# LCSL/nys-koop-lqr

Measured on AMD Instinct MI355X. Metric: Nyström-Koopman fits/sec (K_nm build + A,B,C solve), N=1e5 m=2000 d=384, higher is better.
Workload: dtype f64

## Files before the change

nys_koop_lqr_amd/csrc/nk_api.hip:

```cpp
#include "nk_common.h"
#include "nk_api_internal.h"

#include <cmath>
#include <cstdarg>
#include <cstdio>
#include <cstring>
#include <cstdlib>
#include <algorithm>
#include <mutex>
#include <set>

namespace nk {

static thread_local std::string g_err;

void set_error(const char* fmt, ...) {
  char buf[1024];
  va_list ap;
  va_start(ap, fmt);
  vsnprintf(buf, sizeof(buf), fmt, ap);
  va_end(ap);
  g_err = buf;
}

// ... 334 lines not shown
  NK_TRY(launch_copy2d(ctx, a.ptr, a.ld, mdl->A, mp, m, m));
  if (p > 0) {
    NK_TRY(stage_in(ctx, B, p, m, p, &b));
    NK_TRY(launch_copy2d(ctx, b.ptr, b.ld, mdl->B, mp, m, p));
  }
  NK_TRY(stage_in(ctx, C, m, d, m, &c));
  NK_TRY(launch_copy2d(ctx, c.ptr, c.ld, mdl->C, m, d, m));
  if (W) {
    NK_TRY(stage_in(ctx, W, mp, d, mp, &w));
    NK_TRY(launch_copy2d(ctx, w.ptr, w.ld, mdl->W, mp, d, mp));
  } else {
    NK_TRY(launch_gemm(ctx, false, false, d, mp, m, 1.0, mdl->C, m, mdl->A, mp, 0.0, mdl->W, mp));
  }
  mdl->has_ops = true;
  return NK_OK;
}

static hipError_t copy_ops_block(double* dst, int64_t ldd, const double* src, int64_t lds, int64_t rows, int64_t cols,
                                 hipStream_t st) {
  const hipMemcpyKind kind = is_device_ptr(dst) ? hipMemcpyDeviceToDevice : hipMemcpyDeviceToHost;
  if (ldd == cols && lds == cols) return hipMemcpyAsync(dst, src, (size_t)rows * cols * 8, kind, st);
  return hipMemcpy2DAsync(dst, (size_t)ldd * 8, src, (size_t)lds * 8, (size_t)cols * 8, (size_t)rows, kind, st);
}

extern "C" {

int nk_version(void) { return NK_ABI_VERSION; }

const char* nk_last_error(void) { return g_err.c_str(); }

int nk_device_count(void) {
  int n = 0;
  if (hipGetDeviceCount(&n) != hipSuccess) {
    (void)hipGetLastError();
    return 0;
  }
  return n;
}

int nk_create(int device, nk_ctx** out) {
  NK_REQUIRE(out != nullptr, "nk_create: null output pointer");
  *out = nullptr;
  int n = nk_device_count();
  if (n <= 0) {
    set_error("no HIP device visible: libnyskoop has no CPU fallback");
    return NK_ERR_NO_DEVICE;
  }
  NK_REQUIRE(device >= 0 && device < n, "nk_create: device %d out of range (0..%d)", device, n - 1);
  NK_HIP(hipSetDevice(device));
  hipDeviceProp_t prop;
  NK_HIP(hipGetDeviceProperties(&prop, device));
  if (strncmp(prop.gcnArchName, "gfx950", 6) != 0) {
    set_error("device %d is %s; libnyskoop is built for gfx950 (MI355X) only", device, prop.gcnArchName);
    return NK_ERR_NO_DEVICE;
  }
  nk_ctx* ctx = new nk_ctx();
  ctx->device = device;
  ctx->num_cu = prop.multiProcessorCount;
  int prio_lo = 0, prio_hi = 0;
  NK_HIP(hipDeviceGetStreamPriorityRange(&prio_lo, &prio_hi));
  const int prio_mid = (prio_lo - prio_hi >= 2) ? (prio_lo + prio_hi) / 2 : prio_hi;
  NK_HIP(hipStreamCreateWithPriority(&ctx->stream_main, hipStreamNonBlocking, prio_mid));
  NK_HIP(hipStreamCreateWithPriority(&ctx->stream_side, hipStreamNonBlocking, prio_lo));
  NK_HIP(hipStreamCreateWithPriority(&ctx->stream_prep, hipStreamNonBlocking, prio_hi));
  NK_HIP(hipStreamCreateWithFlags(&ctx->stream_copy, hipStreamNonBlocking));
  NK_HIP(hipStreamCreateWithPriority(&ctx->stream_la[0], hipStreamNonBlocking, prio_hi));
  NK_HIP(hipStreamCreateWithPriority(&ctx->stream_la[1], hipStreamNonBlocking, prio_mid));
  for (int q = 0; q < 2; ++q)
    for (int i = 0; i < 4; ++i) NK_HIP(hipEventCreateWithFlags(&ctx->ev_la[q][i], hipEventDisableTiming));
  ctx->stream = ctx->stream_main;
  ctx->cur_arena = &ctx->arena;
  NK_HIP(hipEventCreateWithFlags(&ctx->ev_fork, hipEventDisableTiming));
  NK_HIP(hipEventCreateWithFlags(&ctx->ev_join, hipEventDisableTiming));
  NK_HIP(hipEventCreateWithFlags(&ctx->ev_chain, hipEventDisableTiming));
  NK_HIP(hipMalloc(reinterpret_cast<void**>(&ctx->d_info), 256));
  ctx->d_piv = reinterpret_cast<unsigned long long*>(ctx->d_info + 16);
  NK_HIP(hipMalloc(reinterpret_cast<void**>(&ctx->d_scalars), HS_COUNT * sizeof(double)));
  NK_HIP(hipHostMalloc(reinterpret_cast<void**>(&ctx->h_scalars), HS_COUNT * sizeof(double), hipHostMallocMapped | hipHostMallocCoherent));
  NK_HIP(hipHostMalloc(reinterpret_cast<void**>(&ctx->h_info), 256, hipHostMallocMapped | hipHostMallocCoherent));
  ctx->h_piv = reinterpret_cast<unsigned long long*>(ctx->h_info + 16);
  for (int i = 0; i < EV_COUNT; ++i) NK_HIP(hipEventCreate(&ctx->ev[i]));
  NK_HIP(hipEventCreateWithFlags(&ctx->ev_ext, hipEventDisableTiming));
  for (int i = 0; i < 8; ++i) NK_HIP(hipEventCreateWithFlags(&ctx->ev_up[i], hipEventDisableTiming));
  const char* km = getenv("NYSKOOP_KMAT");
  ctx->kmat_mode = (km && strcmp(km, "direct") == 0) ? 1 : 0;
  const char* st = getenv("NYSKOOP_STRICT_SPD");
  ctx->strict_spd = (st && atoi(st) != 0) ? 1 : 0;
  if (const char* rp = getenv("NYSKOOP_REFINE_PIVOT")) ctx->refine_pivot = atof(rp);
  if (const char* rs = getenv("NYSKOOP_REFINE_STEPS")) ctx->refine_steps = std::max(0, atoi(rs));
  {
    std::lock_guard<std::mutex> lk(g_reg_mu);
    g_ctxs.insert(ctx);
  }
  *out = ctx;
  return NK_OK;
}

static void destroy_ctx_unregistered(nk_ctx* ctx) {
  (void)hipSetDevice(ctx->device);
  if (tl_ctx == ctx) tl_ctx = nullptr;
  group_detach(ctx);
  (void)hipStreamSynchronize(ctx->stream_main);
  (void)hipStreamSynchronize(ctx->stream_side);
  (void)hipStreamSynchronize(ctx->stream_prep);
  (void)hipStreamSynchronize(ctx->stream_copy);
  for (int q = 0; q < 2; ++q) {
    if (ctx->stream_la[q]) { (void)hipStreamSynchronize(ctx->stream_la[q]); (void)hipStreamDestroy(ctx->stream_la[q]); }
    for (int i = 0; i < 4; ++i) if (ctx->ev_la[q][i]) (void)hipEventDestroy(ctx->ev_la[q][i]);
  }
  for (auto& c : ctx->arena.chunks) (void)hipFree(c.base);
  for (auto& c : ctx->arena_side.chunks) (void)hipFree(c.base);
  (void)hipEventDestroy(ctx->ev_fork);
  (void)hipEventDestroy(ctx->ev_join);
  if (ctx->ev_chain) (void)hipEventDestroy(ctx->ev_chain);
  if (ctx->ev_ext) (void)hipEventDestroy(ctx->ev_ext);
  for (int i = 0; i < 8; ++i) if (ctx->ev_up[i]) (void)hipEventDestroy(ctx->ev_up[i]);
  (void)hipStreamDestroy(ctx->stream_side);
  (void)hipStreamDestroy(ctx->stream_prep);
  (void)hipStreamDestroy(ctx->stream_copy);
  (void)hipFree(ctx->d_info);
  for (int i = 0; i < 2; ++i) if (ctx->d_flow[i]) (void)hipFree(ctx->d_flow[i]);
  (void)hipFree(ctx->d_scalars);
  if (ctx->d_zeros) (void)hipFree(ctx->d_zeros);
  if (ctx->h_stage) (void)hipHostFree(ctx->h_stage);
  (void)hipHostFree(ctx->h_scalars);
  (void)hipHostFree(ctx->h_info);
  for (int i = 0; i < EV_COUNT; ++i) (void)hipEventDestroy(ctx->ev[i]);
  (void)hipStreamDestroy(ctx->stream_main);
  delete ctx;
}

int nk_destroy(nk_ctx* ctx) {
  if (!ctx) return NK_OK;
  {
    std::lock_guard<std::mutex> lk(g_reg_mu);
    if (g_ctxs.erase(ctx) == 0) return NK_OK;
  }
  destroy_ctx_unregistered(ctx);
  return NK_OK;
}

static int model_wait_unchecked(nk_model* mdl);
static void destroy_model_unregistered(nk_model* model, bool to_pool) {
  (void)model_wait_unchecked(model);
  if (to_pool) {
    pool_give(model->device, model->bytes, model->buf);
  } else {
    (void)hipSetDevice(model->device);
    (void)hipFree(model->buf);
  }
  delete model;
}

int nk_shutdown(void) {
  tl_ctx = nullptr;
  std::set<nk_ctx*> ctxs;
  std::set<nk_model*> models;
  std::set<void*> blocks;
  {
    std::lock_guard<std::mutex> lk(g_reg_mu);
    ctxs.swap(g_ctxs);
    models.swap(g_models);
    blocks.swap(g_host_blocks);
  }
  for (nk_ctx* c : ctxs) {
    (void)hipSetDevice(c->device);
    (void)hipStreamSynchronize(c->stream_main);
    (void)hipStreamSynchronize(c->stream_side);
    (void)hipStreamSynchronize(c->stream_prep);
    (void)hipStreamSynchronize(c->stream_copy);
  }
  for (nk_model* m : models) destroy_model_unregistered(m, false);
  for (nk_ctx* c : ctxs) destroy_ctx_unregistered(c);
  pool_drain();
  for (void* b : blocks) (void)hipHostFree(b);
  return NK_OK;
}

int nk_set_compute_dtype(nk_ctx* ctx, int dtype) {
  NK_REQUIRE(ctx != nullptr && (dtype == NK_DTYPE_F64 || dtype == NK_DTYPE_F32), "nk_set_compute_dtype: bad argument");
  ctx->compute_f32 = dtype == NK_DTYPE_F32 ? 1 : 0;
  return NK_OK;
}

int nk_set_strict_spd(nk_ctx* ctx, int strict) {
  NK_REQUIRE(ctx != nullptr && strict >= 0 && strict <= 2, "nk_set_strict_spd: bad argument");
  ctx->strict_spd = strict;
  return NK_OK;
}

int nk_set_refine(nk_ctx* ctx, double pivot_ratio, int32_t steps) {
  NK_REQUIRE(ctx != nullptr && pivot_ratio >= 0.0 && pivot_ratio <= 1.0 && steps >= 0 && steps <= 8, "nk_set_refine: bad argument");
  ctx->refine_pivot = pivot_ratio;
  ctx->refine_steps = steps;
  return NK_OK;
}

int nk_wait_stream(nk_ctx* ctx, void* producer_stream) {
  NK_REQUIRE(ctx != nullptr, "nk_wait_stream: null context");
// ... 271 lines not shown
```

nys_koop_lqr_amd/csrc/nk_common.h:

```cpp
#pragma once
#include <hip/hip_runtime.h>
#include <stdint.h>
#include <stddef.h>
#include <string>
#include <vector>

#include "nyskoop.h"
#include "nk_lockstep.h"
#include "nk_gemm_plan.h"

namespace nk {

void set_error(const char* fmt, ...);

#define NK_HIP(call)                                                                         \
  do {                                                                                       \
    hipError_t e_ = (call);                                                                  \
    if (e_ != hipSuccess) {                                                                  \
      nk::set_error("%s failed: %s (%s:%d)", #call, hipGetErrorString(e_), __FILE__, __LINE__); \
      return e_ == hipErrorOutOfMemory ? NK_ERR_OOM : NK_ERR_HIP;                            \
    }                                                                                        \
  } while (0)

#define NK_TRY(call)            \
  do {                          \
    int rc_ = (call);           \
    if (rc_ != NK_OK) return rc_; \
  } while (0)

#define NK_REQUIRE(cond, ...)     \
  do {                            \
    if (!(cond)) {                \
      nk::set_error(__VA_ARGS__); \
      return NK_ERR_BAD_ARG;      \
    }                             \
  } while (0)

struct ArenaChunk {
  char* base = nullptr;
  size_t cap = 0;
  size_t off = 0;
};
struct Arena {
  std::vector<ArenaChunk> chunks;
  int cur = 0;
};
struct ArenaMark {
  int chunk;
  size_t off;
};

}

enum {
  EV_FIT_BEGIN = 0,
  EV_STAGED = 1,
  EV_KMAT_DONE = 2,
  EV_GRAM_DONE = 3,
  EV_SOLVE_BEGIN = 4,
  EV_FIT_END = 5,
  EV_SQRT_BEGIN = 6,
  EV_SQRT_END = 7,
  EV_LANDMARKS = 8,
  EV_SQRT_PREPARED = 9,
  EV_SQRT_RESID = 10,
  EV_SQRT_SCALARS = 11,
  EV_FORK = 12,
  EV_YPREP_DONE = 13,
  EV_GEMM_T0 = 14,
  EV_GEMM_T1 = 15,
  EV_COUNT = 16
};

enum {
  HS_SCRATCH = 0,
  HS_SQRT_FLAG = 8,
  HS_SQRT_RESID_AT_FLAG = 9,
  HS_SQRT_RESID_LAST = 10,
  HS_SQRT_C = 12,
  HS_SQRT_SUMSQ = 13,
  HS_SQRT_TRACE = 14,
  HS_REFINE = 16,
  HS_COUNT = 64
};
enum {
  SQ_C = 0,
  SQ_SUMSQ = 1,
  SQ_TRACE = 2,
  SQ_LINV2 = 3,
  SQ_FLAG = 5,
  SQ_RESID_AT_FLAG = 6,
  SQ_RESID_LAST = 7,
  SQ_COUNT = 8
};

struct nk_member_state;
struct nk_ctx {
  int device = 0;
  hipStream_t stream = nullptr;
  hipStream_t stream_main = nullptr;
  hipStream_t stream_side = nullptr;
  hipStream_t stream_copy = nullptr;
  hipStream_t stream_prep = nullptr;
  nk::Arena arena;
  nk::Arena arena_side;
  nk::Arena* cur_arena = nullptr;
  hipStream_t stream_la[2] = {nullptr, nullptr};
  hipEvent_t ev_la[2][4] = {};
  int compute_f32 = 0;
  hipEvent_t ev_fork = nullptr, ev_join = nullptr, ev_chain = nullptr;
  int* d_info = nullptr;
  unsigned long long* d_piv = nullptr;
  unsigned long long* h_piv = nullptr;
  double* d_scalars = nullptr;
  double* h_scalars = nullptr;
  int* h_info = nullptr;
  double* d_zeros = nullptr;
  hipEvent_t ev[EV_COUNT];
  int num_cu = 256;
  int kmat_mode = 0;
  double refine_pivot = 0.0;
  int refine_steps = 2;
  int strict_spd = 0;
  hipEvent_t ev_ext = nullptr;
  hipEvent_t ev_up[8] = {};
  nk_group* group = nullptr;
  nk_member_state* gstate = nullptr;
  int* d_flow[2] = {nullptr, nullptr};
  size_t flow_words[2] = {0, 0};
  bool spline_defer_svd = false;
  bool chol_flow_off = false;
  double* h_stage = nullptr;
  size_t h_stage_bytes = 0;
};

enum { NK_MODEL_NYSTROM = 0, NK_MODEL_SPLINE = 1 };
struct nk_model {
  int device = 0;
  int32_t m = 0, d = 0, p = 0;
  int32_t ktype = 0;
  double sigma0 = 0.0;
  double jitter = 0.0;
  double* buf = nullptr;
  size_t bytes = 0;
  double *A = nullptr, *B = nullptr, *C = nullptr, *W = nullptr, *S = nullptr, *Sinv = nullptr, *Z = nullptr,
         *winv = nullptr;
  bool has_ops = false;
  int32_t kind = 0;
  hipEvent_t ev_fetch = nullptr;
};

namespace nk {

struct SideScope {
  nk_ctx* c;
  hipStream_t s0;
  Arena* a0;
  explicit SideScope(nk_ctx* ctx, hipStream_t s = nullptr) : c(ctx), s0(ctx->stream), a0(ctx->cur_arena) {
    c->stream = s ? s : c->stream_side;
    c->cur_arena = &c->arena_side;
  }
  ~SideScope() {
    c->stream = s0;
    c->cur_arena = a0;
  }
};

struct ChainOnly {
  nk_ctx* c;
  bool b0;
  explicit ChainOnly(nk_ctx* ctx) : c(ctx), b0(ctx->chol_flow_off) { c->chol_flow_off = true; }
  ~ChainOnly() { c->chol_flow_off = b0; }
};

inline int info_base(const nk_ctx* c) { return c->stream != c->stream_main ? 2 : 0; }

__device__ __forceinline__ double exp_nonpos_ca() {
  double ca = __longlong_as_double(0x3e5ade156a5dcb37LL);
  asm volatile("" : "+v"(ca));
  return ca;
}
__device__ __forceinline__ double exp_nonpos(double x, double ca_v) {
  const double k = __builtin_rint(x * __longlong_as_double(0x3ff71547652b82feLL));
  double r = __builtin_fma(__longlong_as_double((long long)0xbfe62e42fefa39efULL), k, x);
  r = __builtin_fma(__longlong_as_double((long long)0xbc7abc9e3b39803fULL), k, r);
  double p;
#define NK_EXP_STEP(c) asm("v_fma_f64 %0, %1, %2, %3" : "=v"(p) : "v"(r), "v"(p), "s"(c))
  asm("v_fma_f64 %0, %1, %2, %3" : "=v"(p) : "v"(r), "v"(ca_v), "s"(__longlong_as_double(0x3e928af3fca7ab0cLL)));
  NK_EXP_STEP(__longlong_as_double(0x3ec71dee623fde64LL));
  NK_EXP_STEP(__longlong_as_double(0x3efa01997c89e6b0LL));
  NK_EXP_STEP(__longlong_as_double(0x3f2a01a014761f6eLL));
  NK_EXP_STEP(__longlong_as_double(0x3f56c16c1852b7b0LL));
  NK_EXP_STEP(__longlong_as_double(0x3f81111111122322LL));
  NK_EXP_STEP(__longlong_as_double(0x3fa55555555502a1LL));
  NK_EXP_STEP(__longlong_as_double(0x3fc5555555555511LL));
  NK_EXP_STEP(__longlong_as_double(0x3fe000000000000bLL));
#undef NK_EXP_STEP
  p = __builtin_fma(r, p, 1.0);
  p = __builtin_fma(r, p, 1.0);
  return x < -1075.0 ? 0.0 : ldexp(p, (int)k);
}
__device__ __forceinline__ double exp_nonpos(double x) { return exp_nonpos(x, exp_nonpos_ca()); }

__host__ __device__ __forceinline__ double log_pos(double x) {
#pragma clang fp contract(off)
  const double ln2_hi = 6.93147180369123816490e-01, ln2_lo = 1.90821492927058770002e-10;
  const double Lg1 = 6.666666666666735130e-01, Lg2 = 3.999999999940941908e-01, Lg3 = 2.857142874366239149e-01,
               Lg4 = 2.222219843214978396e-01, Lg5 = 1.818357216161805012e-01, Lg6 = 1.531383769920937332e-01,
               Lg7 = 1.479819860511658591e-01;
  uint64_t bits;
  __builtin_memcpy(&bits, &x, 8);
  int32_t hx = (int32_t)(bits >> 32);
  int k = 0;
  if (hx < 0x00100000) {
    x *= 1.80143985094819840000e+16;
    k -= 54;
    __builtin_memcpy(&bits, &x, 8);
    hx = (int32_t)(bits >> 32);
  }
  k += (hx >> 20) - 1023;
  hx &= 0x000fffff;
  const int32_t i = (hx + 0x95f64) & 0x100000;
  bits = ((uint64_t)(uint32_t)(hx | (i ^ 0x3ff00000)) << 32) | (bits & 0xffffffffULL);
  __builtin_memcpy(&x, &bits, 8);
  k += i >> 20;
  const double f = x - 1.0;
  const double dk = (double)k;
  if ((0x000fffff & (2 + hx)) < 3) {
    if (f == 0.0) return k == 0 ? 0.0 : dk * ln2_hi + dk * ln2_lo;
    const double R = f * f * (0.5 - 0.33333333333333333 * f);
    return k == 0 ? f - R : dk * ln2_hi - ((R - dk * ln2_lo) - f);
  }
  const double s = f / (2.0 + f);
  const double z = s * s;
  const double w = z * z;
  const double t1 = w * (Lg2 + w * (Lg4 + w * Lg6));
  const double t2 = z * (Lg1 + w * (Lg3 + w * (Lg5 + w * Lg7)));
  const double R = t2 + t1;
  if (((hx - 0x6147a) | (0x6b851 - hx)) > 0) {
    const double hfsq = 0.5 * f * f;
    return k == 0 ? f - (hfsq - s * (hfsq + R)) : dk * ln2_hi - ((hfsq - (s * (hfsq + R) + dk * ln2_lo)) - f);
  }
  return k == 0 ? f - s * (f - R) : dk * ln2_hi - ((s * (f - R) - dk * ln2_lo) - f);
}
__host__ __device__ __forceinline__ double tps_value(double r2) {
#pragma clang fp contract(off)
  return r2 > 0.0 ? r2 * log_pos(sqrt(r2)) : 0.0;
}

nk_group* group_new(int device, int size);
void group_attach(nk_group* g, int slot, nk_ctx* c);
void group_detach(nk_ctx* c);
int group_enter(nk_ctx* c);
int group_leave(nk_ctx* c);
void group_stats(nk_ctx* c, uint64_t out[4]);
enum { CNT_CHAIN_GIVEUP = 0, CNT_JACOBI_GIVEUP = 1, CNT_RANK_TRUNCATED = 2, CNT_SQRT_RETRY = 3, CNT_REFINED = 4,
       CNT_CHOL_FLOW_GIVEUP = 5, CNT_CHOL_FLOW = 6, CNT_N = 7 };
void count_event(int which);
uint64_t read_counter(int which);
hipError_t real_stream_sync(hipStream_t s);
hipError_t real_event_sync(hipEvent_t e);

int arena_reset(nk_ctx* ctx);
ArenaMark arena_mark(nk_ctx* ctx);
void arena_release(nk_ctx* ctx, ArenaMark mk);
int arena_alloc(nk_ctx* ctx, size_t bytes, void** out);
template <typename T>
inline int arena_alloc_t(nk_ctx* ctx, size_t count, T** out) {
  return arena_alloc(ctx, count * sizeof(T), reinterpret_cast<void**>(out));
}
bool is_device_ptr(const void* p);

template <typename... Fn>
inline hipError_t dynamic_lds_register(int bytes, Fn*... kernels) {
  hipError_t e = hipSuccess;
  for (const void* f : {reinterpret_cast<const void*>(kernels)...})
    if (e == hipSuccess) e = hipFuncSetAttribute(f, hipFuncAttributeMaxDynamicSharedMemorySize, bytes);
  return e;
}
inline int dynamic_lds_status(hipError_t e) {
  if (e == hipSuccess) return NK_OK;
  set_error("hipFuncSetAttribute(hipFuncAttributeMaxDynamicSharedMemorySize) failed: %s", hipGetErrorString(e));
  return NK_ERR_HIP;
}

struct GemmTimer {
  nk_ctx* ctx;
  float* ms;
  int mark(int slot) const {
    if (ms) NK_HIP(hipEventRecord(ctx->ev[slot], ctx->stream));
    return NK_OK;
  }
  int begin() const { return mark(EV_GEMM_T0); }
  int end() const { return mark(EV_GEMM_T1); }
  int read(bool sync) const {
    if (!ms || !sync) return NK_OK;
    NK_HIP(hipEventSynchronize(ctx->ev[EV_GEMM_T1]));
    NK_HIP(hipEventElapsedTime(ms, ctx->ev[EV_GEMM_T0], ctx->ev[EV_GEMM_T1]));
    return NK_OK;
  }
};

int launch_kmat(nk_ctx* ctx, int ktype, const double* A, int64_t lda, int64_t nA, const double* B, int64_t ldb,
                int64_t nB, int d, const double* winv, double sigma0, double* out, int64_t ldo);

struct GemmOpts {
  int tri = TRI_FULL;
  int splitk = 0;
};
int launch_gemm(nk_ctx* ctx, bool transA, bool transB, int64_t M, int64_t N, int64_t K, double alpha, const double* A,
                int64_t lda, const double* B, int64_t ldb, double beta, double* C, int64_t ldc,
                const GemmOpts& opts = GemmOpts(), float* ms_kernel = nullptr);

struct GemmCall {
  int64_t M = 0, N = 0, K = 0;
  double alpha = 1.0, beta = 0.0;
  const double* A = nullptr;
  const double* B = nullptr;
  double* C = nullptr;
  int64_t lda = 0, ldb = 0, ldc = 0;
  GemmOpts opts;
};
int launch_gemm_pair(nk_ctx* ctx, bool transA, bool transB, const GemmCall* calls, int ncalls);

struct TnSkip;
static inline int grid_for(int64_t total, int num_cu) {
  int64_t b = (total + 255) / 256;
  const int64_t cap = (int64_t)num_cu * 8;
  return (int)(b < 1 ? 1 : (b > cap ? cap : b));
}
int launch_add_diag(nk_ctx* ctx, double* A, int64_t lda, int n, double v);
int launch_copy2d(nk_ctx* ctx, const double* src, int64_t lds, double* dst, int64_t ldd, int64_t rows, int64_t cols);
int launch_axpby2d(nk_ctx* ctx, double a, const double* X, int64_t ldx, double b, double* Y, int64_t ldy,
                   int64_t rows, int64_t cols);
int launch_scale_add_identity(nk_ctx* ctx, double a, const double* X, int64_t ldx, double c, double* Y, int64_t ldy,
                              int n, const TnSkip* skip = nullptr);
int launch_fill(nk_ctx* ctx, double* A, int64_t lda, int64_t rows, int64_t cols, double v);
int launch_frob_minus_identity(nk_ctx* ctx, const double* M, int64_t ldm, int n, double* d_out,
                               const TnSkip* skip = nullptr);
int launch_frob_mi_partials(nk_ctx* ctx, const double* M, int64_t ldm, int n, double* partial, int* count, const TnSkip* skip);
int launch_max_abs_rowsum(nk_ctx* ctx, const double* M, int64_t ldm, int n, double* d_out);
// ... 255 lines not shown
```

nys_koop_lqr_amd/csrc/nk_group.hip:

```cpp
#define NK_LOCKSTEP_NO_MACROS
#include "nk_common.h"

#include <algorithm>
#include <atomic>
#include <condition_variable>
#include <cstdio>
#include <cstdlib>
#include <cstring>
#include <map>
#include <mutex>
#include <unordered_map>

namespace nk {

thread_local nk_ctx* tl_ctx = nullptr;

struct TwinInfo {
  const void* twin;
  size_t bytes;
  const char* name;
};
static std::unordered_map<const void*, TwinInfo>& twin_map() {
  static std::unordered_map<const void*, TwinInfo> m;
  return m;
// ... 357 lines not shown
      (kind == hipMemcpyDeviceToDevice || (kind == hipMemcpyDeviceToHost && bytes <= 512 && ctx_pinned_mirror(c, dst, bytes)))) {
    const int64_t n = (int64_t)(bytes / 4);
    const int64_t blocks = (n + 1023) / 1024;
    ArgPack<const uint32_t*, uint32_t*, int64_t> pk;
    memset(static_cast<void*>(&pk), 0, sizeof(pk));
    pack_fill(pk, static_cast<const uint32_t*>(src), static_cast<uint32_t*>(dst), n);
    std::vector<uint32_t> offs;
    pack_offsets(pk, reinterpret_cast<const char*>(&pk), offs);
    (void)group_record_kernel(c, reinterpret_cast<const void*>(copy_words_kernel), dim3((unsigned)(blocks < 1 ? 1 : (blocks > 2048 ? 2048 : blocks))),
                              dim3(256), 0, &pk, sizeof(pk), offs);
    return hipSuccess;
  }
  GroupOp op;
  op.kind = OP_MEMCPY; op.dst = dst; op.src = src; op.bytes = bytes; op.mk = kind;
  st(c)->ops.push_back(op);
  return hipSuccess;
}
hipError_t x_memcpy2d_async(void* dst, size_t dpitch, const void* src, size_t spitch, size_t width, size_t height,
                            hipMemcpyKind kind, hipStream_t s) {
  nk_ctx* c = rec_ctx();
  if (!c) return hipMemcpy2DAsync(dst, dpitch, src, spitch, width, height, kind, s);
  GroupOp op;
  op.kind = OP_MEMCPY2D; op.dst = dst; op.src = src; op.dpitch = dpitch; op.spitch = spitch; op.width = width;
  op.height = height; op.mk = kind;
  st(c)->ops.push_back(op);
  return hipSuccess;
}
hipError_t x_memset_async(void* dst, int value, size_t bytes, hipStream_t s) {
  nk_ctx* c = rec_ctx();
  if (!c) return hipMemsetAsync(dst, value, bytes, s);
  GroupOp op;
  op.kind = OP_MEMSET; op.dst = dst; op.value = value; op.bytes = bytes;
  st(c)->ops.push_back(op);
  return hipSuccess;
}
hipError_t x_stream_sync(hipStream_t s) {
  nk_ctx* c = rec_ctx();
  if (!c) return hipStreamSynchronize(s);
  return group_sync(c) == NK_OK ? hipSuccess : hipErrorUnknown;
}
hipError_t x_event_sync(hipEvent_t e) {
  nk_ctx* c = rec_ctx();
  if (!c) return hipEventSynchronize(e);
  return group_sync(c) == NK_OK ? hipSuccess : hipErrorUnknown;
}
hipError_t x_event_record(hipEvent_t e, hipStream_t s) {
  if (rec_ctx()) return hipSuccess;
  return hipEventRecord(e, s);
}
hipError_t x_stream_wait_event(hipStream_t s, hipEvent_t e, unsigned flags) {
  if (rec_ctx()) return hipSuccess;
  return hipStreamWaitEvent(s, e, flags);
}
hipError_t x_event_elapsed(float* ms, hipEvent_t a, hipEvent_t b) {
  if (rec_ctx()) {
    if (ms) *ms = 0.f;
    return hipSuccess;
  }
  return hipEventElapsedTime(ms, a, b);
}

nk_group* group_new(int device, int size) {
  nk_group* g = new nk_group();
  g->device = device;
  g->members.assign((size_t)size, nullptr);
  g->live = size;
  if (hipStreamCreateWithFlags(&g->stream, hipStreamNonBlocking) != hipSuccess) { delete g; return nullptr; }
  g->tab_cap = (size_t)8 << 20;
  if (hipHostMalloc(reinterpret_cast<void**>(&g->h_tab), g->tab_cap, hipHostMallocDefault) != hipSuccess ||
      hipMalloc(reinterpret_cast<void**>(&g->d_tab), g->tab_cap) != hipSuccess) {
    if (g->h_tab) (void)hipHostFree(g->h_tab);
    (void)hipStreamDestroy(g->stream);
    delete g;
    return nullptr;
  }
  return g;
}
void group_attach(nk_group* g, int slot, nk_ctx* c) {
  g->members[(size_t)slot] = c;
  c->group = g;
  c->gstate = new nk_member_state();
}
static std::atomic<uint64_t> g_counters[CNT_N];
void count_event(int which) { if (which >= 0 && which < CNT_N) g_counters[which].fetch_add(1, std::memory_order_relaxed); }
uint64_t read_counter(int which) { return g_counters[which].load(std::memory_order_relaxed); }
hipError_t real_stream_sync(hipStream_t s) { return hipStreamSynchronize(s); }
hipError_t real_event_sync(hipEvent_t e) { return hipEventSynchronize(e); }
hipStream_t group_stream(nk_group* g) { return g->stream; }
void group_detach(nk_ctx* c) {
  nk_group* g = c->group;
  if (!g) return;
  bool last = false;
  {
    std::unique_lock<std::mutex> lk(g->mu);
    nk_member_state* s = st(c);
    if (!s->ops.empty()) (void)flush_and_sync_locked(g, std::vector<nk_ctx*>{c});
    if (s->entered) { s->entered = false; g->active--; }
    for (auto& m : g->members) if (m == c) m = nullptr;
    last = --g->live == 0;
    if (!last && g->active > 0 && g->waiting >= g->active) {
      const std::vector<nk_ctx*> ready = waiting_members(g);
      const int rc = flush_and_sync_locked(g, ready);
      release_waiters_locked(g, ready, rc);
      g->cv.notify_all();
    }
  }
  delete c->gstate;
  c->gstate = nullptr;
  c->group = nullptr;
  if (last) {
    (void)hipStreamSynchronize(g->stream);
    (void)hipFree(g->d_tab);
    (void)hipHostFree(g->h_tab);
    (void)hipStreamDestroy(g->stream);
    delete g;
  }
}
int group_enter(nk_ctx* c) {
  nk_group* g = c->group;
  if (!g) return NK_OK;
  std::lock_guard<std::mutex> lk(g->mu);
  if (!st(c)->entered) { st(c)->entered = true; g->active++; }
  return NK_OK;
}
int group_leave(nk_ctx* c) {
  nk_group* g = c->group;
  if (!g) return NK_OK;
  std::unique_lock<std::mutex> lk(g->mu);
  nk_member_state* s = st(c);
  if (!s->entered) return NK_OK;
  int rc_own = NK_OK;
  if (!s->ops.empty())
    rc_own = flush_and_sync_locked(g, std::vector<nk_ctx*>{c});
  s->entered = false;
  g->active--;
  if (g->active > 0 && g->at_align >= g->active) {
    g->at_align = 0;
    g->align_gen++;
  }
  if (g->active > 0 && g->waiting >= g->active) {
    const std::vector<nk_ctx*> ready = waiting_members(g);
    const int rc = flush_and_sync_locked(g, ready);
    release_waiters_locked(g, ready, rc);
    lk.unlock();
    g->cv.notify_all();
  }
  return rc_own;
}
void group_stats(nk_ctx* c, uint64_t out[4]) {
  nk_group* g = c->group;
  out[0] = out[1] = out[2] = out[3] = 0;
  if (!g) return;
  std::lock_guard<std::mutex> lk(g->mu);
  out[0] = g->n_flush; out[1] = g->n_launch_merged; out[2] = g->n_launch_single; out[3] = g->n_units_merged;
}

}
```

nys_koop_lqr_amd/csrc/nk_sqrt_schedule.h:

```cpp
#pragma once
#include <cmath>

namespace nk {

inline double ns_p3(double x) { return x * (3.0 - x) * (3.0 - x) * 0.25; }

inline double ns_interval_estimate(double fro, double tr, int m) {
  double a_lo;
  const double lam1 = fro < 1.0 ? fro : 1.0;
  if (m > 1 && tr > lam1) a_lo = (tr - lam1) / (m - 1);
  else a_lo = tr / m * 1e-2;
  if (!(a_lo > 0.0) || !std::isfinite(a_lo)) a_lo = 1e-12;
  if (a_lo > 1.0) a_lo = 1.0;
  return a_lo;
}

inline double ns_scale(double a, double b) { return 3.0 / (a + std::sqrt(a * b) + b); }

inline void ns_advance(double s2, double& a, double& b) {
  const double xa = s2 * a, xb = s2 * b;
  const double lo = ns_p3(xa) < ns_p3(xb) ? ns_p3(xa) : ns_p3(xb);
  b = (xa <= 1.0 && xb >= 1.0) ? 1.0 : (ns_p3(xa) > ns_p3(xb) ? ns_p3(xa) : ns_p3(xb));
  a = lo < b ? lo : b;
}

constexpr int NS_MAX_STEPS = 100;
struct NsSchedule {
  int kmax = 0;
  double s2[128];
  bool check[128];
};
inline NsSchedule ns_queued_schedule(double estimate, double true_lower) {
  NsSchedule sch;
  double ta = true_lower, tb = 1.0;
  if (ta > estimate) ta = estimate;
  const double a_sched = std::pow(estimate, 0.8) * std::pow(ta, 0.2);
  double a = a_sched, b = 1.0;
  int kconv = -1;
  for (int k = 0; k < NS_MAX_STEPS; ++k) {
    if (kconv < 0 && ta >= 1.0 - 1e-9 && tb <= 1.0 + 1e-9) kconv = k;
    sch.check[k] = a >= 0.5;
    const double s2 = ns_scale(a, b);
    sch.s2[k] = s2;
    ns_advance(s2, a, b);
    ns_advance(s2, ta, tb);
    if (kconv >= 0 && k >= kconv + 1) { sch.kmax = k + 1; break; }
  }
  if (sch.kmax == 0) sch.kmax = NS_MAX_STEPS;
  return sch;
}

}
```

nys_koop_lqr_amd/csrc/nk_sqrtm.hip:

```cpp
#include "nk_common.h"
#include "nk_tn.h"
#include "nk_sqrt_schedule.h"

#include <algorithm>
#include <cmath>

namespace nk {

static int read_scalar(nk_ctx* ctx, const double* d_ptr, double* out) {
  NK_HIP(hipMemcpyAsync(ctx->h_scalars + HS_SCRATCH, d_ptr, sizeof(double), hipMemcpyDeviceToHost, ctx->stream));
  NK_HIP(hipStreamSynchronize(ctx->stream));
  *out = ctx->h_scalars[HS_SCRATCH];
  return NK_OK;
}

struct CoupledBufs {
  double *Y = nullptr, *Z = nullptr, *Yn = nullptr, *Zn = nullptr, *M = nullptr, *T = nullptr;
  double *Yt = nullptr, *Zt = nullptr, *Ytn = nullptr, *Ztn = nullptr;
};

static int coupled_products(nk_ctx* ctx, int m, int it, CoupledBufs& b) {
  TnProblem pr[2];
  pr[0].A = b.Yt; pr[0].B = b.T; pr[0].C = b.Yn; pr[0].lda = pr[0].ldb = pr[0].ldc = m; pr[0].M = pr[0].N = m;
  pr[0].Ct = b.Ytn; pr[0].ldct = m;
// ... 65 lines not shown
    if (a_lo >= 0.5 || it + 1 == maxit) {
      NK_TRY(launch_frob_minus_identity(ctx, b.M, m, m, ctx->d_scalars));
      double r2 = 0.0;
      NK_TRY(read_scalar(ctx, ctx->d_scalars, &r2));
      r_prev = r;
      r = std::sqrt(r2 / m);
      if (!std::isfinite(r)) break;
      if (r < 5e-14 || r_prev < 1e-7) {
        ok = true;
        break;
      }
    }
    const double s2 = ns_scale(a_lo, b_hi);
    const double sc = std::sqrt(s2);
    ns_advance(s2, a_lo, b_hi);
    NK_TRY(launch_scale_add_identity(ctx, -0.5 * s2 * sc, b.M, m, 1.5 * sc, b.T, m, m));
    NK_TRY(coupled_products(ctx, m, it, b));
  }
  if (iters) *iters = it;
  if (resid) *resid = r;
  NK_TRY(x_align());
  if (!ok) {
    set_error("sqrtm: Newton-Schulz did not converge (residual %g after %d iterations)", r, it);
    arena_release(ctx, mk);
    return NK_ERR_NO_CONVERGENCE;
  }
  const double sc = std::sqrt(c);
  NK_TRY(launch_axpby2d(ctx, sc, b.Y, m, 0.0, S, m, m, m));
  NK_TRY(launch_axpby2d(ctx, 1.0 / sc, b.Z, m, 0.0, Sinv, m, m, m));
  arena_release(ctx, mk);
  return NK_OK;
}

__device__ __forceinline__ void tri_scale_both_kernel_body(const double* __restrict__ L, int64_t ldl, int m, const double* __restrict__ d_c, double* __restrict__ Xt, double* __restrict__ X) {
  __shared__ double tile[32][33];
  const double s = 1.0 / sqrt(d_c[0]);
  const int bx = blockIdx.x * 32, by = blockIdx.y * 32;
  const int tx = threadIdx.x & 31, ty = threadIdx.x >> 5;
  for (int r = ty; r < 32; r += 8) {
    const int i = by + r, j = bx + tx;
    double v = 0.0;
    if (i < m && j <= i) v = L[(int64_t)i * ldl + j] * s;
    if (i < m && j < m) Xt[(int64_t)i * m + j] = v;
    tile[r][tx] = v;
  }
  __syncthreads();
  for (int r = ty; r < 32; r += 8) {
    const int i = bx + r, j = by + tx;
    if (i < m && j < m) X[(int64_t)i * m + j] = tile[tx][r];
  }
}
__global__ void __launch_bounds__(256) tri_scale_both_kernel(const double* __restrict__ L, int64_t ldl, int m, const double* __restrict__ d_c, double* __restrict__ Xt, double* __restrict__ X) { tri_scale_both_kernel_body(L, ldl, m, d_c, Xt, X); }
NK_BATCHED_TWIN(tri_scale_both_kernel, (256), const double*, int64_t, int, const double*, double*, double*)

int sqrtm_prepare(nk_ctx* ctx, const double* P, int64_t ldp, int m, SqrtPlan* plan) {
  plan->P = P; plan->ldp = ldp; plan->m = m;
  plan->mark = arena_mark(ctx);
  const size_t mm = (size_t)m * m;
  const int nblk = (m + CHOL_NB - 1) / CHOL_NB;
  NK_TRY(arena_alloc_t(ctx, 2 * mm, &plan->W));
  NK_TRY(arena_alloc_t(ctx, (size_t)nblk * CHOL_WS, &plan->Linv));
  NK_TRY(arena_alloc_t(ctx, mm, &plan->X0));
  NK_TRY(arena_alloc_t(ctx, mm, &plan->X0t));
  NK_TRY(arena_alloc_t(ctx, (size_t)SQ_COUNT, &plan->d_sc));
  NK_TRY(launch_max_abs_rowsum(ctx, P, ldp, m, plan->d_sc + SQ_C));
  NK_TRY(launch_sumsq_trace(ctx, P, ldp, m, plan->d_sc + SQ_SUMSQ, plan->d_sc + SQ_TRACE));
  NK_HIP(hipMemcpyAsync(ctx->h_scalars + HS_SQRT_C, plan->d_sc + SQ_C, 3 * sizeof(double), hipMemcpyDeviceToHost, ctx->stream));
  NK_HIP(hipEventRecord(ctx->ev[EV_SQRT_SCALARS], ctx->stream));
  double* E = plan->W + mm;
  NK_TRY(launch_copy2d(ctx, P, ldp, plan->W, m, m, m));
  NK_TRY(launch_fill(ctx, E, m, m, m, 0.0));
  NK_TRY(launch_add_diag(ctx, E, m, m, 1.0));
  CholSys y;
  y.P = plan->W; y.ldp = m; y.m = m; y.extra = m; y.backward = false; y.Linv = plan->Linv;
  NK_TRY(cholesky_aug_pair_async(ctx, &y, 1, plan->pause_event, plan->pause_step));
  NK_TRY(launch_sumsq_trace(ctx, E, (int64_t)m, m, plan->d_sc + SQ_LINV2, nullptr));
  const int tb = (m + 31) / 32;
  hipLaunchKernelGGL(tri_scale_both_kernel, dim3(tb, tb), dim3(256), 0, ctx->stream, plan->W, (int64_t)m, m, plan->d_sc + SQ_C,
                     plan->X0t, plan->X0);
  NK_HIP(hipGetLastError());
  return NK_OK;
}

__device__ __forceinline__ void ns_flag_kernel_body(const double* __restrict__ partial, int count, int m, int step, double* __restrict__ state) {
  __shared__ double sh[4];
  double s = 0.0;
  for (int i = threadIdx.x; i < count; i += blockDim.x) s += partial[i];
  s = wave_sum(s);
  if ((threadIdx.x & 63) == 0) sh[threadIdx.x >> 6] = s;
  __syncthreads();
  if (threadIdx.x == 0) {
    const double r = sqrt((sh[0] + sh[1] + sh[2] + sh[3]) / m);
    state[2] = r;
    if (state[0] == 0.0 && r < 1e-7) {
      state[0] = (double)(step + 1);
      state[1] = r;
    }
  }
}
__global__ void __launch_bounds__(256) ns_flag_kernel(const double* __restrict__ partial, int count, int m, int step, double* __restrict__ state) { ns_flag_kernel_body(partial, count, m, step, state); }
NK_BATCHED_TWIN(ns_flag_kernel, (256), const double*, int, int, int, double*)

static int sqrtm_polar_products(nk_ctx* ctx, SqrtPlan* plan, const double* Q, double* scratch, double c, double* S,
                                double* Sinv, const double* Q_even = nullptr, const double* select = nullptr) {
  const int m = plan->m;
  const size_t mm = (size_t)m * m;
  double* Linv_full = scratch;
  NK_TRY(launch_transpose(ctx, plan->W + mm, m, Linv_full, m, m, m));
  TnProblem pr[2];
  pr[0].A = Q; pr[0].B = plan->X0; pr[0].C = S; pr[0].lda = pr[0].ldb = pr[0].ldc = m; pr[0].M = pr[0].N = m;
  pr[0].alpha = std::sqrt(c);
  pr[0].ktrim = KTRIM_B_UPPER;
  pr[1].ktrim = KTRIM_A_LOWER;
  pr[1].A = Linv_full; pr[1].B = Q; pr[1].C = Sinv; pr[1].lda = pr[1].ldb = pr[1].ldc = m; pr[1].M = pr[1].N = m;
  pr[0].A_even = Q_even;
  pr[1].B_even = Q_even;
  TnSkip sel;
  sel.select = select;
  if (tn_fast_ok(pr[0]) && tn_fast_ok(pr[1]) && m >= 128) {
    NK_TRY(launch_gemm_tn_multi(ctx, pr, 2, m, 0, nullptr, true, select ? &sel : nullptr));
  } else {
    NK_TRY(launch_gemm(ctx, true, false, m, m, m, pr[0].alpha, Q, m, plan->X0, m, 0.0, S, m));
    NK_TRY(launch_gemm(ctx, true, false, m, m, m, 1.0, Linv_full, m, Q, m, 0.0, Sinv, m));
  }
  return NK_OK;
}

struct SqrtScalars {
  double c = 0.0, sumsq = 0.0, trace = 0.0, linv2 = 0.0;
};

static int scalars_early(nk_ctx* ctx, SqrtPlan* plan, SqrtScalars* sc) {
  NK_HIP(hipEventSynchronize(ctx->ev[EV_SQRT_SCALARS]));
  sc->c = ctx->h_scalars[HS_SQRT_C]; sc->sumsq = ctx->h_scalars[HS_SQRT_SUMSQ]; sc->trace = ctx->h_scalars[HS_SQRT_TRACE];
  if (!(sc->c > 0.0) || !std::isfinite(sc->c)) plan->early = false;
  return NK_OK;
}

static int scalars_synchronous(nk_ctx* ctx, SqrtPlan* plan, int ib, SqrtScalars* sc) {
  NK_HIP(hipMemcpyAsync(ctx->h_scalars + HS_SCRATCH, plan->d_sc, 4 * sizeof(double), hipMemcpyDeviceToHost, ctx->stream));
  NK_HIP(hipMemcpyAsync(ctx->h_info + ib, ctx->d_info + ib, sizeof(int), hipMemcpyDeviceToHost, ctx->stream));
  NK_HIP(hipStreamSynchronize(ctx->stream));
  const double* h = ctx->h_scalars + HS_SCRATCH;
  sc->c = h[SQ_C]; sc->sumsq = h[SQ_SUMSQ]; sc->trace = h[SQ_TRACE]; sc->linv2 = h[SQ_LINV2];
  return NK_OK;
}

static int sqrtm_again_on_chain(nk_ctx* ctx, SqrtPlan* plan, double* S, double* Sinv) {
  count_event(CNT_CHOL_FLOW_GIVEUP);
  arena_release(ctx, plan->mark);
  ChainOnly chain(ctx);
  SqrtPlan again;
  NK_TRY(sqrtm_prepare(ctx, plan->P, plan->ldp, plan->m, &again));
  const int rc = sqrtm_finish(ctx, &again, S, Sinv);
  *plan = again;
  return rc;
}

static int sqrtm_coupled_fallback(nk_ctx* ctx, SqrtPlan* plan, double* S, double* Sinv) {
  arena_release(ctx, plan->mark);
  plan->rc = sqrtm_spd_coupled(ctx, plan->P, plan->ldp, plan->m, S, Sinv, &plan->iters, &plan->resid);
  return plan->rc;
}

struct PolarIter {
  int m = 0;
  double c = 0.0;
  double *Xa = nullptr, *Xta = nullptr, *Xb = nullptr, *Xtb = nullptr, *M = nullptr, *T = nullptr;
  const double *X = nullptr, *Xt = nullptr;
  double *Xn = nullptr, *Xtn = nullptr;
  bool fast = false;
};
static int polar_setup(nk_ctx* ctx, const SqrtPlan* plan, double c, PolarIter* it) {
  const int m = it->m = plan->m;
  const size_t mm = (size_t)m * m;
  it->c = c;
  NK_TRY(arena_alloc_t(ctx, mm, &it->Xa));
  NK_TRY(arena_alloc_t(ctx, mm, &it->Xta));
  NK_TRY(arena_alloc_t(ctx, mm, &it->Xb));
  NK_TRY(arena_alloc_t(ctx, mm, &it->Xtb));
  NK_TRY(arena_alloc_t(ctx, mm, &it->M));
  NK_TRY(arena_alloc_t(ctx, mm, &it->T));
  it->X = plan->X0; it->Xt = plan->X0t;
  it->Xn = it->Xa; it->Xtn = it->Xta;
  TnProblem probe;
  probe.A = it->Xta; probe.B = it->T; probe.C = it->Xa; probe.lda = probe.ldb = probe.ldc = m; probe.M = probe.N = m;
  it->fast = m >= 128 && tn_fast_ok(probe);
  return NK_OK;
}
static int polar_first_m(nk_ctx* ctx, const SqrtPlan* plan, const PolarIter& it) {
  const int m = it.m;
  NK_TRY(launch_transpose(ctx, plan->P, plan->ldp, it.M, m, m, m));
  NK_TRY(launch_axpby2d(ctx, 0.5 / it.c, plan->P, plan->ldp, 0.5 / it.c, it.M, m, m, m));
  return NK_OK;
}
static int polar_x_times_t(nk_ctx* ctx, PolarIter& it, int splitk, const TnSkip* skip) {
  const int m = it.m;
  if (it.fast) {
    TnProblem pr;
    pr.A = it.Xt; pr.B = it.T; pr.C = it.Xn; pr.lda = pr.ldb = pr.ldc = m; pr.M = pr.N = m; pr.Ct = it.Xtn; pr.ldct = m;
    NK_TRY(launch_gemm_tn_multi(ctx, &pr, 1, m, splitk, nullptr, true, skip));
  } else {
    NK_TRY(launch_gemm(ctx, true, false, m, m, m, 1.0, it.Xt, m, it.T, m, 0.0, it.Xn, m));
    NK_TRY(launch_transpose(ctx, it.Xn, m, it.Xtn, m, m, m));
  }
  it.X = it.Xn; it.Xt = it.Xtn;
  it.Xn = (it.Xn == it.Xa) ? it.Xb : it.Xa;
  it.Xtn = (it.Xtn == it.Xta) ? it.Xtb : it.Xta;
  return NK_OK;
}

static int polar_queued(nk_ctx* ctx, SqrtPlan* plan, PolarIter& it, double a_lo, double linv2, double* S, double* Sinv) {
  const int m = it.m;
  const double c = it.c;
  const NsSchedule sch = ns_queued_schedule(a_lo, plan->early ? 0.9 * plan->lambda_min_hint / c : 0.5 / (c * linv2));
  const int kmax = sch.kmax;
  double* state = plan->d_sc + SQ_FLAG;
  NK_HIP(hipMemsetAsync(state, 0, 3 * sizeof(double), ctx->stream));
  double* rpart = nullptr;
  {
    const size_t mt = (size_t)(m + 127) / 128;
    const size_t need = std::max((size_t)grid_for((int64_t)m * m, ctx->num_cu), mt * (mt + 1) / 2 * 8);
    NK_TRY(arena_alloc_t(ctx, need, &rpart));
  }
  for (int k = 0; k < kmax; ++k) {
    TnSkip skip;
    skip.state = state; skip.step = k;
    int npart = 0;
    if (k == 0) {
      NK_TRY(polar_first_m(ctx, plan, it));
    } else {
      const double s2k = sch.s2[k], sck = std::sqrt(s2k);
      TnProblem pm;
      pm.A = it.X; pm.B = it.X; pm.C = it.M; pm.lda = pm.ldb = pm.ldc = m; pm.M = pm.N = m; pm.tri = TRI_UPPER_MIRROR;
      pm.Caff = it.T; pm.aff_a = -0.5 * s2k * sck; pm.aff_c = 1.5 * sck;
      TnSkip skip_m = skip;
      skip_m.resid_partials = rpart; skip_m.resid_count = &npart;
      NK_TRY(launch_gemm_tn_multi(ctx, &pm, 1, m, 0, nullptr, true, &skip_m));
    }
    if (sch.check[k]) {
      if (npart == 0) NK_TRY(launch_frob_mi_partials(ctx, it.M, (int64_t)m, m, rpart, &npart, &skip));
      hipLaunchKernelGGL(ns_flag_kernel, dim3(1), dim3(256), 0, ctx->stream, rpart, npart, m, k, state);
      NK_HIP(hipGetLastError());
    }
    if (k == 0) {
      const double s2 = sch.s2[0], sc = std::sqrt(s2);
      NK_TRY(launch_scale_add_identity(ctx, -0.5 * s2 * sc, it.M, m, 1.5 * sc, it.T, m, m, &skip));
    }
    NK_TRY(polar_x_times_t(ctx, it, 1, &skip));
  }
  NK_TRY(sqrtm_polar_products(ctx, plan, it.Xa, it.T, c, S, Sinv, it.Xb, state));
  NK_HIP(hipMemcpyAsync(ctx->h_scalars + HS_SQRT_FLAG, state, 3 * sizeof(double), hipMemcpyDeviceToHost, ctx->stream));
  if (plan->early)
    NK_HIP(hipMemcpyAsync(ctx->h_info + plan->info_slot, ctx->d_info + plan->info_slot, sizeof(int), hipMemcpyDeviceToHost,
                          ctx->stream));
  plan->deferred = true;
  plan->kmax = kmax;
  arena_release(ctx, plan->mark);
  return NK_OK;
}

static int polar_host_checked(nk_ctx* ctx, SqrtPlan* plan, PolarIter& it, double a_lo, double* S, double* Sinv) {
  const int m = it.m;
  GemmOpts sym;
  sym.tri = TRI_UPPER_MIRROR;
  const int maxit = NS_MAX_STEPS;
  double b_hi = 1.0, r = 1e300;
  int k = 0;
  bool ok = false;
  for (; k < maxit; ++k) {
    if (k == 0) NK_TRY(polar_first_m(ctx, plan, it));
    else NK_TRY(launch_gemm(ctx, true, false, m, m, m, 1.0, it.X, m, it.X, m, 0.0, it.M, m, sym));
    const bool check = a_lo >= 0.5 || k + 2 >= maxit;
    if (check) {
      NK_TRY(launch_frob_minus_identity(ctx, it.M, m, m, ctx->d_scalars));
      NK_HIP(hipMemcpyAsync(ctx->h_scalars + HS_SCRATCH, ctx->d_scalars, sizeof(double), hipMemcpyDeviceToHost, ctx->stream));
      NK_HIP(hipEventRecord(ctx->ev[EV_SQRT_RESID], ctx->stream));
    }
    const double s2 = ns_scale(a_lo, b_hi);
    const double sc = std::sqrt(s2);
    ns_advance(s2, a_lo, b_hi);
    NK_TRY(launch_scale_add_identity(ctx, -0.5 * s2 * sc, it.M, m, 1.5 * sc, it.T, m, m));
    NK_TRY(polar_x_times_t(ctx, it, 0, nullptr));
    if (check) {
      NK_HIP(hipEventSynchronize(ctx->ev[EV_SQRT_RESID]));
      r = std::sqrt(ctx->h_scalars[HS_SCRATCH] / m);
      if (!std::isfinite(r)) break;
      if (r < 1e-7) {
        ok = true;
        ++k;
        break;
      }
    }
  }
  plan->iters = k;
  plan->resid = r;
  NK_TRY(x_align());
  if (!ok) {
    set_error("sqrtm: Newton-Schulz did not converge (residual %g after %d iterations)", r, k);
    arena_release(ctx, plan->mark);
    plan->rc = NK_ERR_NO_CONVERGENCE;
    return plan->rc;
  }
  NK_TRY(sqrtm_polar_products(ctx, plan, it.X, it.T, it.c, S, Sinv));
  arena_release(ctx, plan->mark);
  return NK_OK;
}

int sqrtm_finish(nk_ctx* ctx, SqrtPlan* plan, double* S, double* Sinv) {
  const int m = plan->m;
  const int ib = info_base(ctx);
  plan->deferred = false;
  plan->info_slot = ib;
  plan->rc = NK_OK; plan->iters = 0; plan->resid = 0.0;
  plan->early = plan->lambda_min_hint > 0.0 && m >= 1024 && m % 2 == 0;
  SqrtScalars sc;
  if (plan->early) NK_TRY(scalars_early(ctx, plan, &sc));
  if (!plan->early) {
    NK_TRY(scalars_synchronous(ctx, plan, ib, &sc));
    if (ctx->h_info[ib] == CHOL_FLOW_GIVEUP) return sqrtm_again_on_chain(ctx, plan, S, Sinv);
    const char* hook = getenv("NYSKOOP_SQRT_FORCE_COUPLED");
    const bool forced = hook && hook[0] == '1';
    if (forced || ctx->h_info[ib] != 0 || !(sc.c > 0.0) || !std::isfinite(sc.c) || !(sc.linv2 > 0.0) || !std::isfinite(sc.linv2))
      return sqrtm_coupled_fallback(ctx, plan, S, Sinv);
  }
  PolarIter it;
  NK_TRY(polar_setup(ctx, plan, sc.c, &it));
  const double a_lo = ns_interval_estimate(std::sqrt(sc.sumsq) / sc.c, sc.trace / sc.c, m);
  const bool queued = it.fast && m >= 1024;
  if (plan->early && !queued) {
    set_error("sqrtm: internal: early queueing needs the LDS-DMA path");
    return NK_ERR_BAD_ARG;
  }
// ... 40 lines not shown
```

Baseline: 24.60.

## Bound queued Newton-Schulz steps with a host-polled convergence window

Instead of enqueuing every Newton-Schulz polar iteration up front and relying on device-side skip flags, the host enqueues only a small window past the next convergence check. It then waits on a per-check event and reads a host-mapped word written by the flag kernel, and stops enqueuing once convergence is signaled. This avoids launching and dispatching kernels for steps that would only early-exit. The cost is host synchronization points that can leave the GPU idle between windows, and the path is disabled during graph recording.

```diff
diff --git a/nys_koop_lqr_amd/csrc/nk_api.hip b/nys_koop_lqr_amd/csrc/nk_api.hip
--- a/nys_koop_lqr_amd/csrc/nk_api.hip
+++ b/nys_koop_lqr_amd/csrc/nk_api.hip
@@ -440,6 +440,7 @@
   for (int i = 0; i < EV_COUNT; ++i) NK_HIP(hipEventCreate(&ctx->ev[i]));
   NK_HIP(hipEventCreateWithFlags(&ctx->ev_ext, hipEventDisableTiming));
   for (int i = 0; i < 8; ++i) NK_HIP(hipEventCreateWithFlags(&ctx->ev_up[i], hipEventDisableTiming));
+  for (int i = 0; i < 8; ++i) NK_HIP(hipEventCreateWithFlags(&ctx->ev_step[i], hipEventDisableTiming));
   const char* km = getenv("NYSKOOP_KMAT");
   ctx->kmat_mode = (km && strcmp(km, "direct") == 0) ? 1 : 0;
   const char* st = getenv("NYSKOOP_STRICT_SPD");
@@ -473,6 +474,7 @@
   if (ctx->ev_chain) (void)hipEventDestroy(ctx->ev_chain);
   if (ctx->ev_ext) (void)hipEventDestroy(ctx->ev_ext);
   for (int i = 0; i < 8; ++i) if (ctx->ev_up[i]) (void)hipEventDestroy(ctx->ev_up[i]);
+  for (int i = 0; i < 8; ++i) if (ctx->ev_step[i]) (void)hipEventDestroy(ctx->ev_step[i]);
   (void)hipStreamDestroy(ctx->stream_side);
   (void)hipStreamDestroy(ctx->stream_prep);
   (void)hipStreamDestroy(ctx->stream_copy);
diff --git a/nys_koop_lqr_amd/csrc/nk_common.h b/nys_koop_lqr_amd/csrc/nk_common.h
--- a/nys_koop_lqr_amd/csrc/nk_common.h
+++ b/nys_koop_lqr_amd/csrc/nk_common.h
@@ -81,6 +81,7 @@
   HS_SQRT_SUMSQ = 13,
   HS_SQRT_TRACE = 14,
   HS_REFINE = 16,
+  HS_SQRT_STEP = 24,
   HS_COUNT = 64
 };
 enum {
@@ -124,6 +125,7 @@
   int strict_spd = 0;
   hipEvent_t ev_ext = nullptr;
   hipEvent_t ev_up[8] = {};
+  hipEvent_t ev_step[8] = {};
   nk_group* group = nullptr;
   nk_member_state* gstate = nullptr;
   int* d_flow[2] = {nullptr, nullptr};
@@ -255,8 +257,9 @@
 int group_leave(nk_ctx* c);
 void group_stats(nk_ctx* c, uint64_t out[4]);
 enum { CNT_CHAIN_GIVEUP = 0, CNT_JACOBI_GIVEUP = 1, CNT_RANK_TRUNCATED = 2, CNT_SQRT_RETRY = 3, CNT_REFINED = 4,
-       CNT_CHOL_FLOW_GIVEUP = 5, CNT_CHOL_FLOW = 6, CNT_N = 7 };
+       CNT_CHOL_FLOW_GIVEUP = 5, CNT_CHOL_FLOW = 6, CNT_SQRT_STEPS = 7, CNT_N = 8 };
 void count_event(int which);
+void count_events(int which, uint64_t n);
 uint64_t read_counter(int which);
 hipError_t real_stream_sync(hipStream_t s);
 hipError_t real_event_sync(hipEvent_t e);
diff --git a/nys_koop_lqr_amd/csrc/nk_group.hip b/nys_koop_lqr_amd/csrc/nk_group.hip
--- a/nys_koop_lqr_amd/csrc/nk_group.hip
+++ b/nys_koop_lqr_amd/csrc/nk_group.hip
@@ -463,7 +463,8 @@
   c->gstate = new nk_member_state();
 }
 static std::atomic<uint64_t> g_counters[CNT_N];
-void count_event(int which) { if (which >= 0 && which < CNT_N) g_counters[which].fetch_add(1, std::memory_order_relaxed); }
+void count_events(int which, uint64_t n) { if (which >= 0 && which < CNT_N) g_counters[which].fetch_add(n, std::memory_order_relaxed); }
+void count_event(int which) { count_events(which, 1); }
 uint64_t read_counter(int which) { return g_counters[which].load(std::memory_order_relaxed); }
 hipError_t real_stream_sync(hipStream_t s) { return hipStreamSynchronize(s); }
 hipError_t real_event_sync(hipEvent_t e) { return hipEventSynchronize(e); }
diff --git a/nys_koop_lqr_amd/csrc/nk_sqrt_schedule.h b/nys_koop_lqr_amd/csrc/nk_sqrt_schedule.h
--- a/nys_koop_lqr_amd/csrc/nk_sqrt_schedule.h
+++ b/nys_koop_lqr_amd/csrc/nk_sqrt_schedule.h
@@ -50,4 +50,16 @@
   return sch;
 }
 
+constexpr int NS_WINDOW_DEFAULT = 2;
+constexpr int NS_WINDOW_MAX = 8;
+inline int ns_next_checked(const NsSchedule& sch, int from) {
+  int k = from < 0 ? 0 : from;
+  while (k < sch.kmax && !sch.check[k]) ++k;
+  return k < sch.kmax ? k : sch.kmax;
 }
+inline int ns_window_limit(const NsSchedule& sch, int W, int newest_read) {
+  const int n = ns_next_checked(sch, newest_read + 1) + W;
+  return n < sch.kmax ? n : sch.kmax;
+}
+
+}
diff --git a/nys_koop_lqr_amd/csrc/nk_sqrtm.hip b/nys_koop_lqr_amd/csrc/nk_sqrtm.hip
--- a/nys_koop_lqr_amd/csrc/nk_sqrtm.hip
+++ b/nys_koop_lqr_amd/csrc/nk_sqrtm.hip
@@ -171,7 +171,7 @@
   return NK_OK;
 }
 
-__device__ __forceinline__ void ns_flag_kernel_body(const double* __restrict__ partial, int count, int m, int step, double* __restrict__ state) {
+__device__ __forceinline__ void ns_flag_kernel_body(const double* __restrict__ partial, int count, int m, int step, double* __restrict__ state, double* __restrict__ host_word) {
   __shared__ double sh[4];
   double s = 0.0;
   for (int i = threadIdx.x; i < count; i += blockDim.x) s += partial[i];
@@ -185,10 +185,14 @@
       state[0] = (double)(step + 1);
       state[1] = r;
     }
-  }
-}
-__global__ void __launch_bounds__(256) ns_flag_kernel(const double* __restrict__ partial, int count, int m, int step, double* __restrict__ state) { ns_flag_kernel_body(partial, count, m, step, state); }
-NK_BATCHED_TWIN(ns_flag_kernel, (256), const double*, int, int, int, double*)
+    if (host_word) {
+      *host_word = state[0];
+      __threadfence_system();
+    }
+  }
+}
+__global__ void __launch_bounds__(256) ns_flag_kernel(const double* __restrict__ partial, int count, int m, int step, double* __restrict__ state, double* __restrict__ host_word) { ns_flag_kernel_body(partial, count, m, step, state, host_word); }
+NK_BATCHED_TWIN(ns_flag_kernel, (256), const double*, int, int, int, double*, double*)
 
 static int sqrtm_polar_products(nk_ctx* ctx, SqrtPlan* plan, const double* Q, double* scratch, double c, double* S,
                                 double* Sinv, const double* Q_even = nullptr, const double* select = nullptr) {
@@ -299,45 +303,81 @@
   return NK_OK;
 }
 
+static int sqrt_window() {
+  const char* e = getenv("NYSKOOP_SQRT_WINDOW");
+  const int w = e ? atoi(e) : NS_WINDOW_DEFAULT;
+  return w < 0 ? 0 : (w > NS_WINDOW_MAX ? NS_WINDOW_MAX : w);
+}
+
+struct QueuedIter {
+  NsSchedule sch;
+  double* state = nullptr;
+  double* rpart = nullptr;
+  double* host_word = nullptr;
+};
+
+static int polar_queue_step(nk_ctx* ctx, SqrtPlan* plan, PolarIter& it, const QueuedIter& q, int k) {
+  const int m = it.m;
+  TnSkip skip;
+  skip.state = q.state; skip.step = k;
+  int npart = 0;
+  if (k == 0) {
+    NK_TRY(polar_first_m(ctx, plan, it));
+  } else {
+    const double s2k = q.sch.s2[k], sck = std::sqrt(s2k);
+    TnProblem pm;
+    pm.A = it.X; pm.B = it.X; pm.C = it.M; pm.lda = pm.ldb = pm.ldc = m; pm.M = pm.N = m; pm.tri = TRI_UPPER_MIRROR;
+    pm.Caff = it.T; pm.aff_a = -0.5 * s2k * sck; pm.aff_c = 1.5 * sck;
+    TnSkip skip_m = skip;
+    skip_m.resid_partials = q.rpart; skip_m.resid_count = &npart;
+    NK_TRY(launch_gemm_tn_multi(ctx, &pm, 1, m, 0, nullptr, true, &skip_m));
+  }
+  if (q.sch.check[k]) {
+    if (npart == 0) NK_TRY(launch_frob_mi_partials(ctx, it.M, (int64_t)m, m, q.rpart, &npart, &skip));
+    hipLaunchKernelGGL(ns_flag_kernel, dim3(1), dim3(256), 0, ctx->stream, q.rpart, npart, m, k, q.state, q.host_word);
+    NK_HIP(hipGetLastError());
+    if (q.host_word) NK_HIP(hipEventRecord(ctx->ev_step[k % NS_WINDOW_MAX], ctx->stream));
+  }
+  if (k == 0) {
+    const double s2 = q.sch.s2[0], sc = std::sqrt(s2);
+    NK_TRY(launch_scale_add_identity(ctx, -0.5 * s2 * sc, it.M, m, 1.5 * sc, it.T, m, m, &skip));
+  }
+  NK_TRY(polar_x_times_t(ctx, it, 1, &skip));
+  return NK_OK;
+}
+
 static int polar_queued(nk_ctx* ctx, SqrtPlan* plan, PolarIter& it, double a_lo, double linv2, double* S, double* Sinv) {
   const int m = it.m;
   const double c = it.c;
-  const NsSchedule sch = ns_queued_schedule(a_lo, plan->early ? 0.9 * plan->lambda_min_hint / c : 0.5 / (c * linv2));
-  const int kmax = sch.kmax;
-  double* state = plan->d_sc + SQ_FLAG;
+  QueuedIter q;
+  q.sch = ns_queued_schedule(a_lo, plan->early ? 0.9 * plan->lambda_min_hint / c : 0.5 / (c * linv2));
+  const int kmax = q.sch.kmax;
+  double* state = q.state = plan->d_sc + SQ_FLAG;
   NK_HIP(hipMemsetAsync(state, 0, 3 * sizeof(double), ctx->stream));
-  double* rpart = nullptr;
   {
     const size_t mt = (size_t)(m + 127) / 128;
     const size_t need = std::max((size_t)grid_for((int64_t)m * m, ctx->num_cu), mt * (mt + 1) / 2 * 8);
-    NK_TRY(arena_alloc_t(ctx, need, &rpart));
-  }
-  for (int k = 0; k < kmax; ++k) {
-    TnSkip skip;
-    skip.state = state; skip.step = k;
-    int npart = 0;
-    if (k == 0) {
-      NK_TRY(polar_first_m(ctx, plan, it));
-    } else {
-      const double s2k = sch.s2[k], sck = std::sqrt(s2k);
-      TnProblem pm;
-      pm.A = it.X; pm.B = it.X; pm.C = it.M; pm.lda = pm.ldb = pm.ldc = m; pm.M = pm.N = m; pm.tri = TRI_UPPER_MIRROR;
-      pm.Caff = it.T; pm.aff_a = -0.5 * s2k * sck; pm.aff_c = 1.5 * sck;
-      TnSkip skip_m = skip;
-      skip_m.resid_partials = rpart; skip_m.resid_count = &npart;
-      NK_TRY(launch_gemm_tn_multi(ctx, &pm, 1, m, 0, nullptr, true, &skip_m));
-    }
-    if (sch.check[k]) {
-      if (npart == 0) NK_TRY(launch_frob_mi_partials(ctx, it.M, (int64_t)m, m, rpart, &npart, &skip));
-      hipLaunchKernelGGL(ns_flag_kernel, dim3(1), dim3(256), 0, ctx->stream, rpart, npart, m, k, state);
-      NK_HIP(hipGetLastError());
-    }
-    if (k == 0) {
-      const double s2 = sch.s2[0], sc = std::sqrt(s2);
-      NK_TRY(launch_scale_add_identity(ctx, -0.5 * s2 * sc, it.M, m, 1.5 * sc, it.T, m, m, &skip));
-    }
-    NK_TRY(polar_x_times_t(ctx, it, 1, &skip));
-  }
+    NK_TRY(arena_alloc_t(ctx, need, &q.rpart));
+  }
+  const int W = ctx_recording(ctx) ? 0 : sqrt_window();
+  int queued = 0;
+  if (W == 0) {
+    for (; queued < kmax; ++queued) NK_TRY(polar_queue_step(ctx, plan, it, q, queued));
+  } else {
+    volatile double* word = ctx->h_scalars + HS_SQRT_STEP;
+    *word = 0.0;
+    q.host_word = ctx->h_scalars + HS_SQRT_STEP;
+    for (int read = -1;;) {
+      const int limit = ns_window_limit(q.sch, W, read);
+      for (; queued < limit; ++queued) NK_TRY(polar_queue_step(ctx, plan, it, q, queued));
+      const int next = ns_next_checked(q.sch, read + 1);
+      if (next >= kmax) break;
+      NK_HIP(hipEventSynchronize(ctx->ev_step[next % NS_WINDOW_MAX]));
+      if (*word != 0.0) break;
+      read = next;
+    }
+  }
+  count_events(CNT_SQRT_STEPS, (uint64_t)queued);
   NK_TRY(sqrtm_polar_products(ctx, plan, it.Xa, it.T, c, S, Sinv, it.Xb, state));
   NK_HIP(hipMemcpyAsync(ctx->h_scalars + HS_SQRT_FLAG, state, 3 * sizeof(double), hipMemcpyDeviceToHost, ctx->stream));
   if (plan->early)
```

Result: no change. 24.68, median of 3 (+0.3%).
